# Tencent/FeatherCNN

Hardware: AMD Instinct MI355X
Metric: images/sec fp32 forward @224x224 (higher is better)
Workload: dtype f32; 1 GPU; vgg16 whole net (40 layers in the model file, 20 after fusion level 3), batch 32 per GPU, 224x224x3, fp32, synthetic ...; net=vgg16, mode=net, per_gpu_batch=32, global_batch=32, parallelism=batch-shard x1, launch=hipGraph replay per step, conv_routing=fhip_conv_select_algo_tuned

## Files before the change

feathercnn_amd/_lib.py:

```python
from __future__ import annotations

import collections
import ctypes
import functools
import os

_HERE = os.path.dirname(os.path.abspath(__file__))
_LOADED = {}

STAGE_NAMES = ("wino_input", "wino_gemm", "wino_output", "igemm", "depthwise", "init", "wino_chain")


class fhip_conv_param(ctypes.Structure):
    _fields_ = [(n, ctypes.c_int) for n in (
        "output_channels", "input_channels", "input_h", "input_w", "kernel_h", "kernel_w", "output_h", "output_w",
        "stride_h", "stride_w", "pad_left", "pad_bottom", "pad_right", "pad_top", "group", "bias_term", "activation")]


class fhip_winograd_plan(ctypes.Structure):
    _fields_ = [("tiles_x", ctypes.c_int), ("tiles_y", ctypes.c_int), ("tiles_per_image", ctypes.c_int),
                ("columns", ctypes.c_int), ("columns_padded", ctypes.c_int), ("column_block", ctypes.c_int), ("frequency_points", ctypes.c_int), ("tile_outputs", ctypes.c_int),
                ("in_channels_padded", ctypes.c_int),
                ("out_channels_padded", ctypes.c_int), ("v_offset_bytes", ctypes.c_size_t), ("v_bytes", ctypes.c_size_t),
                ("m_offset_bytes", ctypes.c_size_t), ("m_bytes", ctypes.c_size_t), ("u_bytes", ctypes.c_size_t)]
# ... 63 lines not shown
    "fhip_pooling_output_dim": (_I, [_Q, _PI, _PI]),
    "fhip_pooling": (_I, [_Q, _I, _V, _V, _V]),
    "fhip_softmax": (_I, [_V, _V, _I, _I, _V]),
    "fhip_net_create": (_I, [ctypes.POINTER(_V)]),
    "fhip_net_destroy": (_I, [_V]),
    "fhip_net_set_stream": (_I, [_V, _V]),
    "fhip_net_get_stream": (_I, [_V, ctypes.POINTER(_V)]),
    "fhip_net_set_fusion": (_I, [_V, _I]),
    "fhip_net_set_graph": (_I, [_V, _I]),
    "fhip_net_set_tuned_selection": (_I, [_V, _I]),
    "fhip_net_set_dilated": (_I, [_V, _I]),
    "fhip_net_set_quantized": (_I, [_V, _I]),
    "fhip_net_set_extended_layers": (_I, [_V, _I]),
    "fhip_net_set_concurrency": (_I, [_V, _I]),
    "fhip_net_set_sub_batches": (_I, [_V, _I]),
    "fhip_net_load_param": (_I, [_V, ctypes.c_char_p]),
    "fhip_net_load_param_mem": (_I, [_V, ctypes.c_char_p, _SZ]),
    "fhip_net_load_weights": (_I, [_V, ctypes.c_char_p]),
    "fhip_net_load_weights_mem": (_I, [_V, _V, _SZ]),
    "fhip_net_load_weights_device": (_I, [_V, _V, _SZ]),
    "fhip_net_feed_input": (_I, [_V, ctypes.c_char_p, _I, _I, _I, _I, _V, _I]),
    "fhip_net_feed_pixels": (_I, [_V, ctypes.c_char_p, _I, _V, _I, _I, _I, _I, _I, _V, _V, _I]),
    "fhip_net_feed_yuv420sp": (_I, [_V, ctypes.c_char_p, _I, _V, _I, _I, _I, _I, _I, _I, _V, _V, _I]),
    "fhip_net_feed_pixel_images": (_I, [_V, ctypes.c_char_p, _I, _V, _I, _I, _I, _V, _V, _I]),
    "fhip_net_forward": (_I, [_V]),
    "fhip_net_extract": (_I, [_V, ctypes.c_char_p, ctypes.POINTER(_V), _PI, _PI, _PI, _PI]),
    "fhip_net_extract_host": (_I, [_V, ctypes.c_char_p, _V, _SZ]),
    "fhip_net_layer_count": (_I, [_V]),
    "fhip_net_layer_info": (_I, [_V, _I, ctypes.c_char_p, ctypes.c_char_p, _I, _PI]),
    "fhip_net_layer_conv_param": (_I, [_V, _I, _P, _PI]),
    "fhip_net_layer_fused_pointwise": (_I, [_V, _I, _P, _PI]),
    "fhip_net_layer_chain": (_I, [_V, _I, _PI, _PI]),
    "fhip_net_layer_canvas": (_I, [_V, _I, _PI]),
    "fhip_net_layer_sibling": (_I, [_V, _I, _PI]),
    "fhip_net_layer_residual": (_I, [_V, _I, _PI]),
    "fhip_net_forward_timed": (_I, [_V, ctypes.POINTER(ctypes.c_float)]),
    "fhip_net_memory": (_I, [_V, ctypes.POINTER(_SZ), ctypes.POINTER(_SZ), ctypes.POINTER(_SZ)]),
}

PIXOUT_SIGNATURES = {
    "fhip_pixout_channels": (_I, [_I]),
    "fhip_float_to_pixels": (_I, [_V, _SZ, _V, _I, _I, _I, _I, _I, _I, _V, _V, _V]),
    "fhip_float_to_pixels_host": (_I, [_V, _SZ, _V, _I, _I, _I, _I, _I, _I, _V, _V, _V]),
    "fhip_pixout_last_error": (ctypes.c_char_p, []),
}

GCONV_SIGNATURES = {
    "fhip_gconv_supported": (_I, [_P]),
    "fhip_gconv_get_buffer_size": (_I, [_P, _I, ctypes.POINTER(_SZ), ctypes.POINTER(_SZ)]),
    "fhip_gconv_init": (_I, [_P, _V, _V, _V]),
    "fhip_gconv_forward": (_I, [_P, _I, _V, _V, _V, _V, _V, _V]),
    "fhip_gconv_route": (_I, [_P, _V, _V, ctypes.c_char_p, _I]),
    "fhip_gconv_last_error": (ctypes.c_char_p, []),
}

class fhip_deconv_param(ctypes.Structure):
    _fields_ = [(n, ctypes.c_int) for n in ("output_channels", "input_channels", "input_h", "input_w", "kernel_h", "kernel_w", "output_h", "output_w",
                                            "stride_h", "stride_w", "pad_left", "pad_bottom", "pad_right", "pad_top", "group", "bias_term",
                                            "activation", "output_pad_right", "output_pad_bottom")]


_DP = ctypes.POINTER(fhip_deconv_param)
DECONV_SIGNATURES = {
    "fhip_deconv_assign_output_dim": (_I, [_DP]),
    "fhip_deconv_supported": (_I, [_DP]),
    "fhip_deconv_get_buffer_size": (_I, [_DP, _I, ctypes.POINTER(_SZ), ctypes.POINTER(_SZ)]),
# ... 183 lines not shown
```

feathercnn_amd/csrc/common.h:

```cpp
#pragma once

#include <hip/hip_runtime.h>
#include <stdint.h>

#include "feather_hip/feather_hip.h"

namespace fhip
{

typedef float f32x16 __attribute__((ext_vector_type(16)));
typedef float f32x4 __attribute__((ext_vector_type(4)));

constexpr int kXcds = 8;

int fail(int code, const char* msg);
int fail_hip(hipError_t e, const char* what);

#define FHIP_CHECK_HIP(expr)                                       \
    do                                                             \
    {                                                              \
        hipError_t e__ = (expr);                                   \
        if (e__ != hipSuccess) return ::fhip::fail_hip(e__, #expr); \
    } while (0)

struct StageTimer
{
    StageTimer(int stage, hipStream_t s);
    ~StageTimer();
    int stage;
    hipStream_t stream;
    int slot;
};

int pixel_channels(int type, int* cin, int* cout);
int yuv420sp_check(int type, int w, int h, int target_w, int target_h, int resize_first, int* cout);

int device_compute_units();
size_t device_lds_bytes();

inline int ceil_div(int a, int b) { return (a + b - 1) / b; }
inline int round_up(int a, int b) { return ceil_div(a, b) * b; }
inline size_t round_up_sz(size_t a, size_t b) { return (a + b - 1) / b * b; }

__device__ __forceinline__ int xcd_remap(int bid, int nwg)
{
    const int q = nwg / kXcds, r = nwg % kXcds;
    const int xcd = bid % kXcds, local = bid / kXcds;
    const int start = (xcd < r) ? xcd * (q + 1) : r * (q + 1) + (xcd - r) * q;
    return start + local;
}

__device__ __forceinline__ float apply_act(float v, bool relu) { return relu ? fmaxf(v, 0.f) : v; }

__device__ __forceinline__ float4 ldg4_nt(const float* p)
{
    const f32x4 v = __builtin_nontemporal_load(reinterpret_cast<const f32x4*>(p));
    return make_float4(v.x, v.y, v.z, v.w);
}
__device__ __forceinline__ void stg4_nt(float* p, float4 v)
{
    f32x4 w;
    w.x = v.x;
    w.y = v.y;
    w.z = v.z;
    w.w = v.w;
    __builtin_nontemporal_store(w, reinterpret_cast<f32x4*>(p));
}
#ifndef FHIP_ACT_NT
#define FHIP_ACT_NT 0
#endif
template <int FAMILY>
// ... 55 lines not shown
```

feathercnn_amd/csrc/implicit_gemm.hip:

```cpp
#include <string.h>

#include <algorithm>
#include <mutex>

#include "gemm_core.h"
#include "conv_gemm_policy.h"
#include "dwpw_band.h"
#include "stream_gemm.h"
#include "ip_stream.h"

namespace fhip
{

size_t depthwise_packed_floats(const fhip_conv_param& p, size_t* w12_offset);

using ConvShapeBig = GemmShape<128, 64, 16, 2, 2>;
using ConvShapeSmallM = GemmShape<64, 128, 16, 1, 4>;

static bool conv_small_m(int K) { return K <= 64; }
using ConvShapeNarrow = GemmShape<64, 32, 16, 2, 1, 8>;
static bool conv_narrow_n(long long ntot) { return ntot <= 32; }

static bool stream_eligible(const fhip_conv_param& p)
{
// ... 465 lines not shown
        if (passes <= 3) FHIP_SMALLC_LAUNCH(2, 3);
        else if (passes <= 7) FHIP_SMALLC_LAUNCH(2, 7);
        else FHIP_SMALLC_LAUNCH(2, 11);
    }
#undef FHIP_SMALLC_LAUNCH
    FHIP_CHECK_HIP(hipGetLastError());
    return FHIP_OK;
}

template <class Shape, int MODE, bool TWIN = false>
static void launch(const ConvGemmParams& g0, hipStream_t s)
{
    ConvGemmParams g = g0;
    g.m_tiles = g.Kp / Shape::BM;
    g.n_tiles = ceil_div(g.Ntot, Shape::BN);
    g.batches = g.split_k;
    unsigned grid = (unsigned)(g.batches * g.m_tiles * g.n_tiles);
    if (g.tail_nt0 > 0)
    {
        g.tail_main = g.m_tiles * g.tail_nt0;
        g.part_col0 = g.tail_nt0 * Shape::BN;
        g.part_ntot = (g.n_tiles - g.tail_nt0) * Shape::BN;
        grid = (unsigned)(g.tail_main + g.m_tiles * (g.n_tiles - g.tail_nt0) * g.split_k);
    }
    else
    {
        g.tail_main = 0;
        g.part_col0 = 0;
        g.part_ntot = g.Ntot;
    }
    hipLaunchKernelGGL((gemm_mfma_kernel<Shape, ConvGemmPolicy<MODE, TWIN>>), dim3(grid), dim3(Shape::THREADS), 0, s, g);
}

int igemm_forward(const fhip_conv_param& p, int batch, float* out, const float* in, const float* packed, const float* bias,
                  float* buffer, bool force_no_act, hipStream_t s, const float* residual)
{
    if (p.group > 1) return fail(FHIP_E_UNSUPPORTED, "implicit GEMM handles group == 1 only");
    if (batch < 1) return fail(FHIP_E_BADARG, "batch < 1");
    if (p.bias_term && !bias) return fail(FHIP_E_BADARG, "bias_term set but bias_arr is NULL");
    ConvGemmParams g;
    g.batches = 1;
    g.Wt = packed;
    g.in = in;
    g.out = out;
    g.out2 = nullptr;
    g.twin_rows = g.relu2 = 0;
    g.bias = bias;
    g.has_residual = residual != nullptr;
    g.residual_delta = residual ? reinterpret_cast<const char*>(residual) - reinterpret_cast<const char*>(out) : 0;
    g.C = p.input_channels;
    g.K = p.output_channels;
    g.H = p.input_h;
    g.W = p.input_w;
    g.OH = p.output_h;
    g.OW = p.output_w;
    g.SH = p.stride_h > 0 ? p.stride_h : 1;
    g.SW = p.stride_w > 0 ? p.stride_w : 1;
    g.PL = p.pad_left;
    g.PT = p.pad_top;
    g.KH = p.kernel_h;
    g.KW = p.kernel_w;
    g.Kd = g.C * g.KH * g.KW;
    int kdp;
    igemm_packed_dims(p, &kdp, &g.Kp);
    g.Kdp = kdp;
    g.bm = conv_small_m(g.K) ? 64 : 128;
// ... 20 lines not shown
        q.bias = bias;
        q.C = g.C;
        q.K = g.K;
        q.HW = g.OHW;
        const bool ragged = (g.OHW % 4) != 0;
        q.gpi = (g.OHW + 3) / 4;
        q.total_px = ragged ? (long long)batch * q.gpi * 4 : ntot;
        q.mgroups = g.K / 32;
        q.px_tiles = (int)((q.total_px + 127) / 128);
        const unsigned blocks = (unsigned)q.px_tiles * (unsigned)((q.mgroups + 3) / 4);
        StageTimer tm(FHIP_STAGE_IGEMM, s);
#define FHIP_STREAM(D_, B_, R_)                                                                                     \
    do                                                                                                              \
    {                                                                                                               \
        if (ragged) hipLaunchKernelGGL((stream_gemm_kernel<D_, B_, R_, true>), dim3(blocks), dim3(256), 0, s, q);   \
        else hipLaunchKernelGGL((stream_gemm_kernel<D_, B_, R_, false>), dim3(blocks), dim3(256), 0, s, q);         \
    } while (0)
        const int pick = ((g.C % 32) == 0 ? 4 : 0) | (g.has_bias ? 2 : 0) | (g.relu ? 1 : 0);
        switch (pick)
        {
            case 7: FHIP_STREAM(16, true, true); break;
            case 6: FHIP_STREAM(16, true, false); break;
            case 5: FHIP_STREAM(16, false, true); break;
            case 4: FHIP_STREAM(16, false, false); break;
            case 3: FHIP_STREAM(8, true, true); break;
            case 2: FHIP_STREAM(8, true, false); break;
            case 1: FHIP_STREAM(8, false, true); break;
            default: FHIP_STREAM(8, false, false); break;
        }
#undef FHIP_STREAM
        FHIP_CHECK_HIP(hipGetLastError());
        return FHIP_OK;
    }
    if (!residual && ip_profitable(p, batch))
    {
        if (!buffer) return fail(FHIP_E_BADARG, "this geometry streams its weight matrix in pieces and needs the scratch buffer GetBufferSize asked for");
        IpStreamParams q;
        q.wp = packed + (size_t)kdp * g.Kp + (stream_eligible(p) ? (size_t)g.K * g.C : 0);
        q.xq = buffer;
        q.partial = buffer + ip_xq_floats(p);
        q.K = g.K;
        q.Kg = ip_kg(p);
        q.KQ = ip_kq(p);
        q.S = ip_pieces(p);
        q.batch = batch;
        StageTimer tm(FHIP_STAGE_IGEMM, s);
        hipLaunchKernelGGL(ip_pack_input_kernel, dim3(ceil_div(q.KQ, kIpPackOctets)), dim3(256), 0, s, buffer, in, batch, g.C, q.KQ);
        hipLaunchKernelGGL(ip_stream_kernel<4>, dim3((unsigned)q.S * (unsigned)ceil_div(q.Kg, 4)), dim3(256), 0, s, q);
        hipLaunchKernelGGL(ip_reduce_kernel, dim3(ceil_div(g.K * batch, 256)), dim3(256), 0, s, out, q.partial, bias, g.K, batch, q.S, g.has_bias, g.relu);
        FHIP_CHECK_HIP(hipGetLastError());
        return FHIP_OK;
    }
    g.split_k = igemm_split(p, batch);
    g.tail_main = g.tail_nt0 = 0;
    if (g.split_k <= 1)
    {
        int pieces;
        g.tail_nt0 = igemm_tail(p, batch, &pieces);
        if (g.tail_nt0) g.split_k = pieces;
    }
    if (g.split_k > 1 && !buffer) return fail(FHIP_E_BADARG, "this geometry runs split-K and needs the scratch buffer GetBufferSize asked for");
    g.partial = buffer;
    g.k_tiles = kdp / kConvKTile;
    g.m_tiles = 0;

    const bool one = g.KH == 1 && g.KW == 1 && p.pad_left == 0 && p.pad_right == 0 && p.pad_top == 0 && p.pad_bottom == 0;
    int mode = 0;
    if (one) mode = (g.SH == 1 && g.SW == 1 && (g.OHW % 4) == 0) ? 2 : 1;
    if (ragged_1x1(p, batch))
    {
        mode = 5;
        g.rag_gpi = (g.OHW + 3) / 4;
        const long long slots = igemm_columns(p, batch);
        if (slots > 0x7fffff00LL) return fail(FHIP_E_BADARG, "N*Ho*Wo exceeds 32-bit column indices: more than 0x7fffff00 GEMM columns");
        g.Ntot = (int)slots;
    }
    const bool small = conv_small_m(g.K);
    StageTimer tm(FHIP_STAGE_IGEMM, s);
    if (conv_narrow_n(ntot))
    {
        if (mode == 2) launch<ConvShapeNarrow, 2>(g, s);
        else if (mode == 1) launch<ConvShapeNarrow, 1>(g, s);
        else launch<ConvShapeNarrow, 0>(g, s);
    }
    else if (small)
// ... 219 lines not shown
```

feathercnn_amd/csrc/ip_stream.h:

```cpp
#pragma once

#include "common.h"

namespace fhip
{

struct IpStreamParams
{
    const float* wp;
    const float* xq;
    float* partial;
    int K, Kg, KQ, S, batch;
};

__global__ __launch_bounds__(256) void ip_pack_weights_kernel(float* __restrict__ wp, const float* __restrict__ w, int K, int C, int Kg, int KQ)
{
    const long long i = (long long)blockIdx.x * 256 + threadIdx.x;
    if (i >= (long long)Kg * KQ * 64) return;
    const int lane = (int)(i & 63);
    const long long gq = i >> 6;
    const int q = (int)(gq % KQ), g = (int)(gq / KQ);
    const int m = 32 * g + (lane & 31), k0 = 8 * q + (lane >> 5);
    float v[4];
#pragma unroll
// ... 79 lines not shown
            }
#pragma unroll
            for (int u = 0; u < UNR; ++u)
            {
                av[u] = an[u];
                bv[u] = bn[u];
            }
        }
        a += (size_t)UNR * 64;
        b += (size_t)UNR * 64;
#pragma unroll
        for (int u = 0; u < UNR; ++u)
        {
            FHIP_IP_MFMA4(av[u], bv[u]);
        }
    }
    for (int u = 0; u < tail; ++u)
    {
        const f32x4 a1 = FHIP_IP_LDW(a + (size_t)u * 64), b1 = b[(size_t)u * 64];
        FHIP_IP_MFMA4(a1, b1);
    }
    const int n = lane & 31, half = lane >> 5;
    if (n >= p.batch) return;
    float* out = p.partial + ((size_t)s * p.K + 32 * g + 4 * half) * p.batch + n;
#pragma unroll
    for (int r = 0; r < 16; ++r)
    {
        const int row = (r & 3) + 8 * (r >> 2);
        if (32 * g + 4 * half + row < p.K) out[(size_t)row * p.batch] = acc0[r] + acc1[r];
    }
}
#undef FHIP_IP_MFMA4

__global__ __launch_bounds__(256) void ip_reduce_kernel(float* __restrict__ out, const float* __restrict__ partial, const float* __restrict__ bias, int K,
                                                        int batch, int S, int has_bias, int relu)
{
    const int i = blockIdx.x * 256 + threadIdx.x, total = K * batch;
    if (i >= total) return;
    const int m = i / batch, n = i - m * batch;
    float acc = 0.f;
    int s = 0;
    for (; s + 4 <= S; s += 4)
    {
        const float v0 = partial[(size_t)s * total + i], v1 = partial[(size_t)(s + 1) * total + i], v2 = partial[(size_t)(s + 2) * total + i],
                    v3 = partial[(size_t)(s + 3) * total + i];
        acc = (((acc + v0) + v1) + v2) + v3;
    }
    for (; s < S; ++s) acc += partial[(size_t)s * total + i];
    if (has_bias) acc += bias[m];
    if (relu) acc = fmaxf(acc, 0.f);
    out[(size_t)n * K + m] = acc;
}

}
```

feathercnn_amd/csrc/net.hip:

```cpp
#include "net_side.h"
#include "net_model.h"
#include "net_core.h"
#include "net_conv.h"
#include "net_layers.h"
#include "net_plan.h"

namespace fhip::net
{

static Layer* create_extended_layer(const std::string& type)
{
    if (type == "Interp") return new InterpLayer;
    if (type == "HardSwish") return new HardSwishLayer;
    if (type == "LRN") return new LRNLayer;
    return nullptr;
}

static Layer* create_layer(const std::string& type)
{
    if (type == "Input") return new InputLayer;
    if (type == "Convolution" || type == "ConvolutionDepthWise") return new ConvLayer;
    if (type == "Deconvolution" || type == "DeconvolutionDepthWise") return new DeconvLayer;
    if (type == "ReLU") return new ReluLayer;
    if (type == "InstanceNorm") return new InstanceNormLayer;
// ... 675 lines not shown

int fhip_net_layer_sibling(fhip_net* n, int index, int* state)
{
    NET_GUARD(n);
    if (index < 0 || index >= (int)n->impl.layers.size() || !state) return fail(FHIP_E_BADARG, "layer index out of range");
    *state = n->impl.layers[index]->sibling_state();
    return FHIP_OK;
}

int fhip_net_layer_residual(fhip_net* n, int index, int* state)
{
    NET_GUARD(n);
    if (index < 0 || index >= (int)n->impl.layers.size() || !state) return fail(FHIP_E_BADARG, "layer index out of range");
    *state = n->impl.layers[index]->residual_state();
    return FHIP_OK;
}

int fhip_net_layer_chain(fhip_net* n, int index, int* v_from_previous, int* writes_next_v)
{
    NET_GUARD(n);
    if (index < 0 || index >= (int)n->impl.layers.size() || !v_from_previous || !writes_next_v) return fail(FHIP_E_BADARG, "layer index out of range");
    n->impl.layers[index]->chain_state(v_from_previous, writes_next_v);
    return FHIP_OK;
}

int fhip_net_layer_canvas(fhip_net* n, int index, int* canvas)
{
    NET_GUARD(n);
    if (index < 0 || index >= (int)n->impl.layers.size() || !canvas) return fail(FHIP_E_BADARG, "layer index out of range");
    *canvas = n->impl.layers[index]->canvas_state();
    return FHIP_OK;
}

int fhip_net_forward_timed(fhip_net* n, float* ms)
{
    NET_GUARD(n);
    if (!ms) return fail(FHIP_E_BADARG, "null argument");
    if (!n->more.empty())
        return fail(FHIP_E_UNSUPPORTED, "per-layer timing of a net with sub-batch replicas: kernels of concurrent replicas share the chip, "
                                        "so their durations are not layer times -- time a net created without fhip_net_set_sub_batches");
    Net& net = n->impl;
    int rc = prepare(net);
    if (rc) return rc;
    const size_t L = net.layers.size();
    std::vector<hipEvent_t> ev(L + 1);
    for (auto& e : ev) FHIP_CHECK_HIP(hipEventCreate(&e));
    FHIP_CHECK_HIP(hipEventRecord(ev[0], net.stream));
    for (size_t i = 0; i < L && rc == 0; ++i)
    {
        rc = net.layers[i]->Forward(net.stream);
        (void)hipEventRecord(ev[i + 1], net.stream);
    }
    (void)hipStreamSynchronize(net.stream);
    if (rc == 0)
        for (size_t i = 0; i < L; ++i) (void)hipEventElapsedTime(&ms[i], ev[i], ev[i + 1]);
    for (auto& e : ev) (void)hipEventDestroy(e);
    return rc;
}

int fhip_net_memory(fhip_net* n, size_t* blob_bytes, size_t* weight_bytes, size_t* arena_bytes)
{
    NET_GUARD(n);
    size_t bb = 0, wb = 0;
    for (auto& kv : n->impl.blobs) bb += kv.second->capacity * sizeof(float);
    for (auto& b : n->impl.shadowed) bb += b->capacity * sizeof(float);
    for (auto& l : n->impl.layers) wb += l->weight_bytes();
// ... 18 lines not shown
```

feathercnn_amd/csrc/net_core.h:

```cpp
#pragma once
#include "net_model.h"

namespace fhip::net
{

struct Blob
{
    std::string name;
    int n = 0, c = 0, h = 0, w = 0;
    float* data = nullptr;
    size_t capacity = 0;
    Blob* alias = nullptr;
    bool fused_away = false;
    bool chained = false;

    size_t count() const { return (size_t)n * c * h * w; }
    int reshape(int n_, int c_, int h_, int w_)
    {
        n = n_;
        c = c_;
        h = h_;
        w = w_;
        alias = nullptr;
        if (chained && !data) return 0;
// ... 40 lines not shown
        {
            release();
            FHIP_CHECK_HIP(hipMalloc((void**)&d, std::max<size_t>(count, 1) * 4));
            bytes = count * 4;
        }
        if (count) FHIP_CHECK_HIP(hipMemcpyAsync(d, h, count * 4, hipMemcpyHostToDevice, s));
        return 0;
    }
    int resize(size_t nbytes)
    {
        if (bytes != nbytes)
        {
            release();
            FHIP_CHECK_HIP(hipMalloc((void**)&d, std::max<size_t>(nbytes, 4)));
            bytes = nbytes;
        }
        return 0;
    }
    void release()
    {
        if (d) (void)hipFree(d);
        d = nullptr;
        bytes = 0;
    }
    ~DeviceVec() { release(); }
};

struct Net;
struct ConvLayer;
struct PoolingLayer;
struct AffineLayer;
struct EltwiseLayer;
struct InterpLayer;

struct Layer
{
    std::string type, name;
    std::vector<Blob*> bottoms, tops;
    Net* net = nullptr;

    virtual ~Layer() {}
    virtual bool needs_weights() const { return false; }
    virtual ConvLayer* as_conv() { return nullptr; }
    virtual PoolingLayer* as_pooling() { return nullptr; }
    virtual AffineLayer* as_affine() { return nullptr; }
    virtual EltwiseLayer* as_eltwise() { return nullptr; }
    virtual InterpLayer* as_interp() { return nullptr; }
    virtual const float* relu_slope() const { return nullptr; }
    template <class Api, class Call>
    int side(const Api* api, const Call& call, int code = 0, const char* prefix = "") const
    {
        if (!api) return FHIP_E_UNSUPPORTED;
        const int rc = call(api);
        return rc ? failf(code ? code : rc, "layer %s: %s%s", name.c_str(), prefix, api->last_error()) : 0;
    }
    virtual int LoadParam(const ParamDict&) { return 0; }
    virtual int LoadWeights(ModelBin&) { return 0; }
    virtual int Reshape()
    {
        if (tops.size() != 1 || bottoms.size() != 1) return failf(NET_E_BASE_RESHAPE, "layer %s: base Reshape needs 1 bottom and 1 top", name.c_str());
        return tops[0]->reshape(bottoms[0]->n, bottoms[0]->c, bottoms[0]->h, bottoms[0]->w);
    }
    int reshape_with(const void* side_library) { return side_library ? Layer::Reshape() : FHIP_E_UNSUPPORTED; }
    virtual int Init(hipStream_t) { return 0; }
    virtual int Forward(hipStream_t) = 0;
    virtual int Fuse(Layer*, int ) { return 0; }
    virtual size_t weight_bytes() const { return 0; }
    virtual size_t arena_bytes() const { return 0; }
    virtual int algo() const { return -1; }
    virtual const fhip_conv_param* conv_param() const { return nullptr; }
    virtual const fhip_conv_param* fused_pointwise(int*) const { return nullptr; }
    virtual void chain_state(int* v_from_previous, int* writes_next_v) const { *v_from_previous = *writes_next_v = 0; }
    virtual int canvas_state() const { return 0; }
    virtual int sibling_state() const { return 0; }
    virtual int residual_state() const { return 0; }
};

static bool is_plain_relu(const Layer* l)
{
    const float* slope = l->relu_slope();
    return slope && *slope == 0.f;
// ... 75 lines not shown
```

feathercnn_amd/csrc/net_layers.h:

```cpp
#pragma once
#include "net_conv.h"

namespace fhip::net
{

struct InputLayer : Layer
{
    int Reshape() override { return 0; }
    int Forward(hipStream_t) override { return 0; }
};

struct InnerProductLayer : Layer
{
    fhip_conv_param p;
    size_t input_size = 0, output_size = 0, weight_data_size = 0;
    std::vector<float> w_host, b_host;
    DeviceVec packed, bias;
    size_t buffer_bytes = 0, packed_bytes = 0;
    BuiltFor built;
    bool quant = false;
    QuantRoute qr;

    InnerProductLayer() { memset(&p, 0, sizeof(p)); }
    bool needs_weights() const override { return true; }
    int LoadParam(const ParamDict& pd) override
    {
        output_size = pd.get(0, 0);
        p.bias_term = pd.get(1, 0);
        weight_data_size = pd.get(2, 0);
        if (pd.get(0, 0) < 1) return failf(NET_E_SHAPE, "layer %s: num_output must be positive", name.c_str());
        if (pd.get(2, 0) < 0 || weight_data_size % output_size)
            return failf(NET_E_SHAPE, "layer %s: weight_data_size is no whole number of rows of num_output", name.c_str());
        input_size = weight_data_size / output_size;
        p.input_channels = (int)input_size;
        p.output_channels = (int)output_size;
        p.input_h = p.input_w = p.kernel_h = p.kernel_w = p.stride_h = p.stride_w = p.group = 1;
        fhip_conv_assign_output_dim(&p);
        quant = qr.read_scale_term(pd) != 0 && net && net->quantized;
        if (quant && (qr.scale_term < 0 || qr.scale_term > 100))
            return failf(NET_E_UNKNOWN_LAYER, "layer %s: int8_scale_term %d (requantised int8 output) is not supported", name.c_str(), qr.scale_term);
        return 0;
    }
    int LoadWeights(ModelBin& mb) override
    {
        if (quant) return qr.load(this, mb, weight_data_size, (int)output_size, p.bias_term != 0);
        int rc = mb.load(weight_data_size, 0, w_host);
        if (rc) return rc;
        if (p.bias_term) rc = mb.load(output_size, 1, b_host);
        return rc;
    }
    int Reshape() override
    {
        const Blob* b = bottoms[0];
        const size_t per_image = (size_t)b->c * b->h * b->w;
        if (input_size != per_image)
            return failf(NET_E_SHAPE, "In Layer %s: Bottom %s data size %zu is inconsistant with expected input size %zu.", name.c_str(), b->name.c_str(), per_image, input_size);
        if (quant)
        {
            copy_geometry(qr.q, p);
            return qr.reshape(this);
        }
        int rc = tops[0]->reshape(b->n, (int)output_size, 1, 1);
        if (rc) return rc;
        return fhip_conv_get_buffer_size(&p, FHIP_IM2COL, b->n, &buffer_bytes, &packed_bytes);
    }
    int Init(hipStream_t s) override
    {
        if (quant) return qr.init(this, AffineFold(), s);
        if (built.done()) return 0;
        const int rc = init_main(p, FHIP_IM2COL, w_host, b_host, packed, packed_bytes, bias, s);
        if (rc) return rc;
        std::vector<float>().swap(w_host);
        built = BuiltFor{FHIP_IM2COL, 0, packed_bytes};
        return 0;
    }
    int Forward(hipStream_t s) override
    {
        if (quant) return qr.forward(this, s);
        return fhip_conv_forward(&p, FHIP_IM2COL, bottoms[0]->n, tops[0]->data, bottoms[0]->data, packed.d, (float*)net->arena.d,
                                 p.bias_term ? bias.d : nullptr, s);
    }
    int Fuse(Layer* next, int) override
    {
        if (!is_plain_relu(next)) return 0;
        p.activation = FHIP_ACT_RELU;
        return 1;
    }
    size_t weight_bytes() const override { return packed.bytes + bias.bytes + qr.bytes(); }
    size_t arena_bytes() const override { return buffer_bytes; }
    int algo() const override { return quant ? FHIP_NET_ROUTE_QCONV : FHIP_IM2COL; }
};

struct ReluLayer : Layer
{
    float slope = 0.f;
    int LoadParam(const ParamDict& pd) override
    {
        slope = pd.get(0, 0.f);
        return 0;
    }
    int Reshape() override { return slope == 0.f ? Layer::Reshape() : reshape_with(inorm_api()); }
    int Forward(hipStream_t s) override
    {
        if (slope == 0.f) return fhip_relu(tops[0]->data, bottoms[0]->data, bottoms[0]->count(), s);
        const Blob* b = bottoms[0];
        return side(inorm_api(), [&](const InormApi* api) {
            return api->activation(FHIP_ACTIVATION_LEAKY_RELU, tops[0]->data, b->data, b->n, b->c, b->h * b->w, slope, 0.f, nullptr, s);
        });
    }
    const float* relu_slope() const override { return &slope; }
};
// ... 966 lines not shown
        for (Blob* t : tops) t->share(bottoms[0]);
        return 0;
    }
    int Forward(hipStream_t) override { return 0; }
};

struct DropoutLayer : Layer
{
    float scale = 1.f;
    DeviceVec d_scale;
    int LoadParam(const ParamDict& pd) override
    {
        scale = pd.get(0, 1.f);
        return 0;
    }
    int Reshape() override
    {
        if (scale == 1.f)
        {
            tops[0]->share(bottoms[0]);
            return 0;
        }
        return Layer::Reshape();
    }
    int Init(hipStream_t s) override
    {
        if (scale == 1.f || d_scale.d) return 0;
        std::vector<float> v(bottoms[0]->c, scale);
        int rc = d_scale.upload(v.data(), v.size(), s);
        if (rc) return rc;
        FHIP_CHECK_HIP(hipStreamSynchronize(s));
        return 0;
    }
    int Forward(hipStream_t s) override
    {
        if (scale == 1.f) return 0;
        const Blob* b = bottoms[0];
        return fhip_affine(tops[0]->data, b->data, d_scale.d, nullptr, b->n, b->c, b->h * b->w, 0, s);
    }
};

}
```

feathercnn_amd/csrc/net_plan.h:

```cpp
#pragma once
#include "net_layers.h"

namespace fhip::net
{

static bool is_channel_map_type(const Layer* l)
{
    return l->type == "ShuffleChannel" || l->type == "Slice" || (l->type == "Concat" && static_cast<const ConcatLayer*>(l)->axis == 0);
}

static void collapse_channel_maps(Net& net)
{
    auto holds = [](const std::vector<Blob*>& v, const Blob* b) { return std::find(v.begin(), v.end(), b) != v.end(); };
    for (size_t i = 0; i < net.layers.size(); ++i)
    {
        if (!is_channel_map_type(net.layers[i].get())) continue;
        std::vector<Blob*> made = net.layers[i]->tops;
        size_t end = i + 1;
        for (; end < net.layers.size(); ++end)
        {
            const Layer* l = net.layers[end].get();
            if (!is_channel_map_type(l)) break;
            bool reads = false, sole = true;
            for (const Blob* b : l->bottoms)
// ... 365 lines not shown
    }
    net.chain_slot[0] = 0;
    net.chain_slot[1] = slot[0];
    net.chain_m = slot[0] + slot[1];
    for (ConvLayer* c : conv)
        if (c && c->chain.runs()) c->chain.arena(slot[0] + slot[1] + msz);
    return 0;
}

static int plan_siblings(Net& net)
{
    const size_t L = net.layers.size();
    std::vector<ConvLayer*> conv(L, nullptr);
    for (size_t i = 0; i < L; ++i)
        if (net.layers[i]->type != "ConvolutionDepthWise" && (conv[i] = net.layers[i]->as_conv())) conv[i]->sibs.reset();
    if (net.fusion < 2) return 0;
    auto root = [](const Blob* b) { return b->alias ? b->alias : b; };
    auto plain = [](const ConvLayer* c) { return c && c->unclaimed() && c->algo_ == FHIP_IM2COL && c->tops.size() == 1 && c->bottoms.size() == 1; };
    auto pairs = [&](const ConvLayer* a, const ConvLayer* b) {
        if (!plain(a) || !plain(b) || root(a->bottoms[0]) != root(b->bottoms[0]) || a->tops[0] == b->tops[0]) return false;
        if (a->p.output_channels <= 64 || b->p.output_channels <= 64) return false;
        return fhip_conv_can_fuse_siblings(&a->p, a->algo_, &b->p, b->algo_, a->bottoms[0]->n) != 0;
    };
    for (size_t i = 0; i < L; ++i)
    {
        if (i + 1 < L && pairs(conv[i], conv[i + 1]))
            SiblingPlan::pair(conv[i], conv[i + 1]);
        else if (conv[i])
            conv[i]->sibs.unpaired();
    }
    return 0;
}

static int reshape_all(Net& net)
{
    net.drop_graph();
    size_t need = 0;
    for (auto& l : net.layers)
    {
        const int rc = l->Reshape();
        if (rc) return rc;
    }
    {
        int rc = plan_chains(net);
        if (rc) return rc;
        if ((rc = plan_siblings(net))) return rc;
    }
    for (auto& l : net.layers) need = std::max(need, l->arena_bytes());
    if (need > net.arena.bytes)
    {
        const int rc = net.arena.resize(need);
        if (rc) return rc;
    }
    net.shapes_dirty = false;
    return plan_concurrency(net);
}

static int prepare(Net& net)
{
    if (!net.param_loaded) return failf(NET_E_IO, "Network has not been loaded. Please load the param file first.");
    if (!net.weights_loaded)
    {
        bool needs = false;
        for (auto& l : net.layers) needs = needs || l->needs_weights();
        if (needs) return failf(NET_E_IO, "weights have not been loaded");
    }
    fuse_layers(net);
    for (auto& kv : net.blobs)
        if (!kv.second->fused_away && kv.second->count() == 0)
        {
            bool is_input = false;
            for (auto& l : net.layers)
                if (l->type == "Input")
                    for (Blob* tb : l->tops) is_input = is_input || tb == kv.second.get();
            if (is_input) return failf(NET_E_SHAPE, "input blob %s has not been fed", kv.first.c_str());
        }
    if (net.shapes_dirty)
    {
        const int rc = reshape_all(net);
        if (rc) return rc;
    }
    for (auto& l : net.layers)
    {
        const int rc = l->Init(net.stream);
        if (rc) return rc;
    }
    net.initialized = true;
    return 0;
// ... 52 lines not shown
```

feathercnn_amd/net.py:

```python
from __future__ import annotations

import ctypes

import numpy as np

from . import _lib
from .booster import ALGO_NAMES, FeatherHipError, _check, _stream


ROUTE_GCONV = 100
ROUTE_NAMES = dict(ALGO_NAMES)
ROUTE_NAMES[ROUTE_GCONV] = "GCONV"
ROUTE_DECONV = 101
ROUTE_NAMES[ROUTE_DECONV] = "DECONV"
ROUTE_INORM = 102
ROUTE_NAMES[ROUTE_INORM] = "INORM"
ROUTE_SHUFFLE = 103
ROUTE_NAMES[ROUTE_SHUFFLE] = "SHUFFLE"
ROUTE_ATROUS = 104
ROUTE_NAMES[ROUTE_ATROUS] = "ATROUS"
ROUTE_GATE = 105
ROUTE_NAMES[ROUTE_GATE] = "GATE"
ROUTE_RESAMPLE = 106
ROUTE_NAMES[ROUTE_RESAMPLE] = "RESAMPLE"
# ... 201 lines not shown
        for i in range(self._lib.fhip_net_layer_count(self._h)):
            st = ctypes.c_int()
            if self._lib.fhip_net_layer_sibling(self._h, i, ctypes.byref(st)) == 0 and st.value:
                out[i] = st.value
        return out

    def residuals(self):
        out = {}
        for i in range(self._lib.fhip_net_layer_count(self._h)):
            st = ctypes.c_int()
            if self._lib.fhip_net_layer_residual(self._h, i, ctypes.byref(st)) == 0 and st.value:
                out[i] = st.value
        return out

    def chains(self, raw=False):
        out = {}
        for i in range(self._lib.fhip_net_layer_count(self._h)):
            a, b = ctypes.c_int(), ctypes.c_int()
            if self._lib.fhip_net_layer_chain(self._h, i, ctypes.byref(a), ctypes.byref(b)) == 0 and (a.value or b.value):
                if raw:
                    out[i] = (a.value, b.value)
                elif a.value == 1 or b.value == 1:
                    out[i] = (a.value == 1, b.value == 1)
        return out

    def canvases(self):
        out = []
        for i in range(self._lib.fhip_net_layer_count(self._h)):
            c = ctypes.c_int()
            if self._lib.fhip_net_layer_canvas(self._h, i, ctypes.byref(c)) == 0 and c.value:
                out.append(i)
        return out

    def forward_timed(self):
        n = self._lib.fhip_net_layer_count(self._h)
        ms = (ctypes.c_float * max(n, 1))()
        _check(self._lib.fhip_net_forward_timed(self._h, ms), "fhip_net_forward_timed")
        info = self.layers()
        return [(t, nm, a, ms[i]) for i, (t, nm, a) in enumerate(info)]

    def memory(self):
        v = [ctypes.c_size_t() for _ in range(3)]
        _check(self._lib.fhip_net_memory(self._h, *[ctypes.byref(x) for x in v]), "fhip_net_memory")
        return {"blob_bytes": v[0].value, "weight_bytes": v[1].value, "arena_bytes": v[2].value}


def _p(t):
    return ctypes.c_void_p(t.data_ptr()) if t is not None else None


def relu(x):
    import torch
    y = torch.empty_like(x)
    _check(_lib.load_library().fhip_relu(_p(y), _p(x), x.numel(), _stream()), "fhip_relu")
    return y


def add(a, b, relu: bool = False):
    import torch
    y = torch.empty_like(a)
    _check(_lib.load_library().fhip_add(_p(y), _p(a), _p(b), a.numel(), int(relu), _stream()), "fhip_add")
    return y


def affine(x, mul, add_=None, relu: bool = False):
    import torch
# ... 29 lines not shown
```

include/feather_hip/feather_net.h:

```cpp
#ifndef FEATHER_NET_H_
#define FEATHER_NET_H_

#include "feather_hip/feather_hip.h"

#ifdef __cplusplus
extern "C" {
#endif


FHIP_API int fhip_relu(float* y, const float* x, size_t count, void* stream);

FHIP_API int fhip_add(float* y, const float* a, const float* b, size_t count, int relu, void* stream);

FHIP_API int fhip_affine(float* y, const float* x, const float* mul, const float* add, int batch, int channels, int hw,
                         int relu, void* stream);


enum
{
    FHIP_PIXEL_CONVERT_SHIFT = 16,
    FHIP_PIXEL_RGB = 1,
    FHIP_PIXEL_BGR = (1 << 1),
    FHIP_PIXEL_GRAY = (1 << 2),
    FHIP_PIXEL_RGBA = (1 << 3),
// ... 88 lines not shown
FHIP_API int fhip_net_load_param(fhip_net* net, const char* path);
FHIP_API int fhip_net_load_param_mem(fhip_net* net, const char* text, size_t len);
FHIP_API int fhip_net_load_weights(fhip_net* net, const char* path);
FHIP_API int fhip_net_load_weights_mem(fhip_net* net, const void* data, size_t len);
FHIP_API int fhip_net_load_weights_device(fhip_net* net, const void* device_data, size_t len);

FHIP_API int fhip_net_feed_input(fhip_net* net, const char* blob_name, int n, int c, int h, int w, const float* data,
                                 int on_device);
FHIP_API int fhip_net_feed_pixels(fhip_net* net, const char* blob_name, int n, const unsigned char* pixels, int type, int w, int h,
                                  int target_w, int target_h, const float* mean, const float* norm, int on_device);
FHIP_API int fhip_net_feed_yuv420sp(fhip_net* net, const char* blob_name, int n, const unsigned char* yuv, int w, int h, int target_w,
                                    int target_h, int type, int resize_first, const float* mean, const float* norm, int on_device);
FHIP_API int fhip_net_feed_pixel_images(fhip_net* net, const char* blob_name, int n, const fhip_pixel_image* images, int type,
                                        int target_w, int target_h, const float* mean, const float* norm, int on_device);
FHIP_API int fhip_net_forward(fhip_net* net);
FHIP_API int fhip_net_extract(fhip_net* net, const char* blob_name, float** device_ptr, int* n, int* c, int* h, int* w);
FHIP_API int fhip_net_extract_host(fhip_net* net, const char* blob_name, float* host, size_t capacity);

FHIP_API int fhip_net_layer_count(fhip_net* net);
#define FHIP_NET_ROUTE_GCONV 100
#define FHIP_NET_ROUTE_DECONV 101
#define FHIP_NET_ROUTE_INORM 102
#define FHIP_NET_ROUTE_SHUFFLE 103
#define FHIP_NET_ROUTE_ATROUS 104
#define FHIP_NET_ROUTE_GATE 105
#define FHIP_NET_ROUTE_RESAMPLE 106
#define FHIP_NET_ROUTE_LRN 107
#define FHIP_NET_ROUTE_QCONV 108
FHIP_API int fhip_net_layer_info(fhip_net* net, int index, char* type, char* name, int len, int* algo);
FHIP_API int fhip_net_layer_conv_param(fhip_net* net, int index, fhip_conv_param* param, int* batch);
FHIP_API int fhip_net_layer_fused_pointwise(fhip_net* net, int index, fhip_conv_param* param, int* one_kernel);
FHIP_API int fhip_net_layer_chain(fhip_net* net, int index, int* v_from_previous, int* writes_next_v);
FHIP_API int fhip_net_layer_canvas(fhip_net* net, int index, int* canvas);
FHIP_API int fhip_net_layer_sibling(fhip_net* net, int index, int* state);
FHIP_API int fhip_net_layer_residual(fhip_net* net, int index, int* state);
FHIP_API int fhip_net_forward_timed(fhip_net* net, float* ms);
FHIP_API int fhip_net_memory(fhip_net* net, size_t* blob_bytes, size_t* weight_bytes, size_t* arena_bytes);

#ifdef __cplusplus
}
#endif
#endif
```

Baseline: 10270 images/s.

## Hand over packed inner-product input directly from reduce kernel to next FC layer

When two streaming inner-product layers follow each other (optionally through pass-through layers like dropout), the first layer's reduce kernel now also writes its output in the packed layout the next layer expects. The next layer then skips its input-packing kernel. This removes one kernel launch and a read/write pass per FC pair in VGG16's classifier head. In exchange the reduce kernel does extra scattered stores, and it relies on planning checks so the arena scratch is not clobbered between the two layers.

```diff
diff --git a/feathercnn_amd/_lib.py b/feathercnn_amd/_lib.py
--- a/feathercnn_amd/_lib.py
+++ b/feathercnn_amd/_lib.py
@@ -119,6 +119,7 @@
     "fhip_net_layer_fused_pointwise": (_I, [_V, _I, _P, _PI]),
     "fhip_net_layer_chain": (_I, [_V, _I, _PI, _PI]),
     "fhip_net_layer_canvas": (_I, [_V, _I, _PI]),
+    "fhip_net_layer_handover": (_I, [_V, _I, _PI, _PI]),
     "fhip_net_layer_sibling": (_I, [_V, _I, _PI]),
     "fhip_net_layer_residual": (_I, [_V, _I, _PI]),
     "fhip_net_forward_timed": (_I, [_V, ctypes.POINTER(ctypes.c_float)]),
diff --git a/feathercnn_amd/csrc/common.h b/feathercnn_amd/csrc/common.h
--- a/feathercnn_amd/csrc/common.h
+++ b/feathercnn_amd/csrc/common.h
@@ -37,6 +37,17 @@
 
 int device_compute_units();
 size_t device_lds_bytes();
+
+struct IpHandover
+{
+    bool packed_in = false;
+    float* next_xq = nullptr;
+    int next_kq = 0;
+};
+bool ip_streams(const fhip_conv_param& p, int batch);
+size_t ip_xq_bytes(const fhip_conv_param& p);
+int ip_forward(const fhip_conv_param& p, int batch, float* out, const float* in, const float* packed, const float* bias, float* buffer, hipStream_t s,
+               const IpHandover& h);
 
 inline int ceil_div(int a, int b) { return (a + b - 1) / b; }
 inline int round_up(int a, int b) { return ceil_div(a, b) * b; }
diff --git a/feathercnn_amd/csrc/implicit_gemm.hip b/feathercnn_amd/csrc/implicit_gemm.hip
--- a/feathercnn_amd/csrc/implicit_gemm.hip
+++ b/feathercnn_amd/csrc/implicit_gemm.hip
@@ -521,6 +521,43 @@
     hipLaunchKernelGGL((gemm_mfma_kernel<Shape, ConvGemmPolicy<MODE, TWIN>>), dim3(grid), dim3(Shape::THREADS), 0, s, g);
 }
 
+static int ip_launch(const fhip_conv_param& p, int batch, float* out, const float* in, const float* packed, const float* bias, float* buffer, bool relu,
+                     hipStream_t s, const IpHandover& h)
+{
+    if (!buffer) return fail(FHIP_E_BADARG, "this geometry streams its weight matrix in pieces and needs the scratch buffer GetBufferSize asked for");
+    int kdp, kp;
+    igemm_packed_dims(p, &kdp, &kp);
+    const int K = p.output_channels, C = p.input_channels;
+    IpStreamParams q;
+    q.wp = packed + (size_t)kdp * kp + (stream_eligible(p) ? (size_t)K * C : 0);
+    q.xq = buffer;
+    q.partial = buffer + ip_xq_floats(p);
+    q.K = K;
+    q.Kg = ip_kg(p);
+    q.KQ = ip_kq(p);
+    q.S = ip_pieces(p);
+    q.batch = batch;
+    if (h.next_xq && h.next_kq != ceil_div(K, 8)) return fail(FHIP_E_BADARG, "the next layer's packed input does not have this layer's output width");
+    StageTimer tm(FHIP_STAGE_IGEMM, s);
+    if (!h.packed_in) hipLaunchKernelGGL(ip_pack_input_kernel, dim3(ceil_div(q.KQ, kIpPackOctets)), dim3(256), 0, s, buffer, in, batch, C, q.KQ);
+    hipLaunchKernelGGL(ip_stream_kernel<4>, dim3((unsigned)q.S * (unsigned)ceil_div(q.Kg, 4)), dim3(256), 0, s, q);
+    const int reduce_threads = h.next_xq ? h.next_kq * 256 : K * batch;
+    hipLaunchKernelGGL(ip_reduce_kernel, dim3(ceil_div(reduce_threads, 256)), dim3(256), 0, s, out, q.partial, bias, K, batch, q.S, p.bias_term != 0, relu ? 1 : 0,
+                       h.next_xq, h.next_kq);
+    FHIP_CHECK_HIP(hipGetLastError());
+    return FHIP_OK;
+}
+
+bool ip_streams(const fhip_conv_param& p, int batch) { return ip_profitable(p, batch); }
+size_t ip_xq_bytes(const fhip_conv_param& p) { return ip_xq_floats(p) * sizeof(float); }
+int ip_forward(const fhip_conv_param& p, int batch, float* out, const float* in, const float* packed, const float* bias, float* buffer, hipStream_t s,
+               const IpHandover& h)
+{
+    if (!ip_profitable(p, batch) || !out || !packed || (!in && !h.packed_in)) return fail(FHIP_E_BADARG, "bad argument");
+    if (p.bias_term && !bias) return fail(FHIP_E_BADARG, "bias_term set but bias_arr is NULL");
+    return ip_launch(p, batch, out, in, packed, bias, buffer, p.activation == FHIP_ACT_RELU, s, h);
+}
+
 int igemm_forward(const fhip_conv_param& p, int batch, float* out, const float* in, const float* packed, const float* bias,
                   float* buffer, bool force_no_act, hipStream_t s, const float* residual)
 {
@@ -607,25 +644,7 @@
         FHIP_CHECK_HIP(hipGetLastError());
         return FHIP_OK;
     }
-    if (!residual && ip_profitable(p, batch))
-    {
-        if (!buffer) return fail(FHIP_E_BADARG, "this geometry streams its weight matrix in pieces and needs the scratch buffer GetBufferSize asked for");
-        IpStreamParams q;
-        q.wp = packed + (size_t)kdp * g.Kp + (stream_eligible(p) ? (size_t)g.K * g.C : 0);
-        q.xq = buffer;
-        q.partial = buffer + ip_xq_floats(p);
-        q.K = g.K;
-        q.Kg = ip_kg(p);
-        q.KQ = ip_kq(p);
-        q.S = ip_pieces(p);
-        q.batch = batch;
-        StageTimer tm(FHIP_STAGE_IGEMM, s);
-        hipLaunchKernelGGL(ip_pack_input_kernel, dim3(ceil_div(q.KQ, kIpPackOctets)), dim3(256), 0, s, buffer, in, batch, g.C, q.KQ);
-        hipLaunchKernelGGL(ip_stream_kernel<4>, dim3((unsigned)q.S * (unsigned)ceil_div(q.Kg, 4)), dim3(256), 0, s, q);
-        hipLaunchKernelGGL(ip_reduce_kernel, dim3(ceil_div(g.K * batch, 256)), dim3(256), 0, s, out, q.partial, bias, g.K, batch, q.S, g.has_bias, g.relu);
-        FHIP_CHECK_HIP(hipGetLastError());
-        return FHIP_OK;
-    }
+    if (!residual && ip_profitable(p, batch)) return ip_launch(p, batch, out, in, packed, bias, buffer, g.relu, s, IpHandover());
     g.split_k = igemm_split(p, batch);
     g.tail_main = g.tail_nt0 = 0;
     if (g.split_k <= 1)
diff --git a/feathercnn_amd/csrc/ip_stream.h b/feathercnn_amd/csrc/ip_stream.h
--- a/feathercnn_amd/csrc/ip_stream.h
+++ b/feathercnn_amd/csrc/ip_stream.h
@@ -135,12 +135,9 @@
 }
 #undef FHIP_IP_MFMA4
 
-__global__ __launch_bounds__(256) void ip_reduce_kernel(float* __restrict__ out, const float* __restrict__ partial, const float* __restrict__ bias, int K,
-                                                        int batch, int S, int has_bias, int relu)
+__device__ __forceinline__ float ip_reduce_value(const float* __restrict__ partial, const float* __restrict__ bias, int i, int m, int total, int S, int has_bias,
+                                                 int relu)
 {
-    const int i = blockIdx.x * 256 + threadIdx.x, total = K * batch;
-    if (i >= total) return;
-    const int m = i / batch, n = i - m * batch;
     float acc = 0.f;
     int s = 0;
     for (; s + 4 <= S; s += 4)
@@ -152,7 +149,29 @@
     for (; s < S; ++s) acc += partial[(size_t)s * total + i];
     if (has_bias) acc += bias[m];
     if (relu) acc = fmaxf(acc, 0.f);
-    out[(size_t)n * K + m] = acc;
+    return acc;
+}
+
+__global__ __launch_bounds__(256) void ip_reduce_kernel(float* __restrict__ out, const float* __restrict__ partial, const float* __restrict__ bias, int K,
+                                                        int batch, int S, int has_bias, int relu, float* __restrict__ xq_next, int KQ_next)
+{
+    const int i = blockIdx.x * 256 + threadIdx.x, total = K * batch;
+    if (xq_next)
+    {
+        if (i >= KQ_next * 256) return;
+        const int n = i & 31, m = i >> 5;
+        float v = 0.f;
+        if (n < batch && m < K)
+        {
+            v = ip_reduce_value(partial, bias, m * batch + n, m, total, S, has_bias, relu);
+            out[(size_t)n * K + m] = v;
+        }
+        xq_next[((size_t)(m >> 3) * 64 + n + 32 * (m & 1)) * 4 + ((m & 7) >> 1)] = v;
+        return;
+    }
+    if (i >= total) return;
+    const int m = i / batch, n = i - m * batch;
+    out[(size_t)n * K + m] = ip_reduce_value(partial, bias, i, m, total, S, has_bias, relu);
 }
 
 }
diff --git a/feathercnn_amd/csrc/net.hip b/feathercnn_amd/csrc/net.hip
--- a/feathercnn_amd/csrc/net.hip
+++ b/feathercnn_amd/csrc/net.hip
@@ -731,6 +731,16 @@
     return FHIP_OK;
 }
 
+int fhip_net_layer_handover(fhip_net* n, int index, int* packed_in, int* writes_next)
+{
+    NET_GUARD(n);
+    if (index < 0 || index >= (int)n->impl.layers.size() || !packed_in || !writes_next) return fail(FHIP_E_BADARG, "layer index out of range");
+    const InnerProductLayer* ip = n->impl.layers[index]->as_inner_product();
+    *packed_in = ip && ip->hand.packed_in ? 1 : 0;
+    *writes_next = ip && ip->hand.next_kq ? 1 : 0;
+    return FHIP_OK;
+}
+
 int fhip_net_forward_timed(fhip_net* n, float* ms)
 {
     NET_GUARD(n);
diff --git a/feathercnn_amd/csrc/net_core.h b/feathercnn_amd/csrc/net_core.h
--- a/feathercnn_amd/csrc/net_core.h
+++ b/feathercnn_amd/csrc/net_core.h
@@ -96,6 +96,7 @@
 struct AffineLayer;
 struct EltwiseLayer;
 struct InterpLayer;
+struct InnerProductLayer;
 
 struct Layer
 {
@@ -110,7 +111,9 @@
     virtual AffineLayer* as_affine() { return nullptr; }
     virtual EltwiseLayer* as_eltwise() { return nullptr; }
     virtual InterpLayer* as_interp() { return nullptr; }
+    virtual InnerProductLayer* as_inner_product() { return nullptr; }
     virtual const float* relu_slope() const { return nullptr; }
+    virtual bool passes_through() const { return false; }
     template <class Api, class Call>
     int side(const Api* api, const Call& call, int code = 0, const char* prefix = "") const
     {
diff --git a/feathercnn_amd/csrc/net_layers.h b/feathercnn_amd/csrc/net_layers.h
--- a/feathercnn_amd/csrc/net_layers.h
+++ b/feathercnn_amd/csrc/net_layers.h
@@ -20,9 +20,12 @@
     BuiltFor built;
     bool quant = false;
     QuantRoute qr;
+    IpHandover hand;
 
     InnerProductLayer() { memset(&p, 0, sizeof(p)); }
     bool needs_weights() const override { return true; }
+    InnerProductLayer* as_inner_product() override { return this; }
+    bool streams() const { return !quant && ip_streams(p, bottoms[0]->n); }
     int LoadParam(const ParamDict& pd) override
     {
         output_size = pd.get(0, 0);
@@ -77,6 +80,12 @@
     int Forward(hipStream_t s) override
     {
         if (quant) return qr.forward(this, s);
+        if (hand.packed_in || hand.next_kq)
+        {
+            IpHandover h = hand;
+            if (h.next_kq) h.next_xq = (float*)net->arena.d;
+            return ip_forward(p, bottoms[0]->n, tops[0]->data, bottoms[0]->data, packed.d, p.bias_term ? bias.d : nullptr, (float*)net->arena.d, s, h);
+        }
         return fhip_conv_forward(&p, FHIP_IM2COL, bottoms[0]->n, tops[0]->data, bottoms[0]->data, packed.d, (float*)net->arena.d,
                                  p.bias_term ? bias.d : nullptr, s);
     }
@@ -1109,6 +1118,7 @@
         FHIP_CHECK_HIP(hipStreamSynchronize(s));
         return 0;
     }
+    bool passes_through() const override { return scale == 1.f; }
     int Forward(hipStream_t s) override
     {
         if (scale == 1.f) return 0;
diff --git a/feathercnn_amd/csrc/net_plan.h b/feathercnn_amd/csrc/net_plan.h
--- a/feathercnn_amd/csrc/net_plan.h
+++ b/feathercnn_amd/csrc/net_plan.h
@@ -421,6 +421,36 @@
     return 0;
 }
 
+static void plan_handovers(Net& net)
+{
+    const size_t L = net.layers.size();
+    for (auto& l : net.layers)
+        if (InnerProductLayer* ip = l->as_inner_product()) ip->hand = IpHandover();
+    if (net.fusion < 3) return;
+    auto main_stream = [&](size_t i) { return i >= net.side.size() || net.side[i] < 0; };
+    for (size_t i = 0; i < L; ++i)
+    {
+        InnerProductLayer* a = net.layers[i]->as_inner_product();
+        if (!a || a->tops.size() != 1 || a->bottoms.size() != 1 || !a->streams() || !main_stream(i)) continue;
+        const Blob* t = a->tops[0];
+        int j = readers(net, t, i + 1).sole();
+        while (j >= 0 && net.layers[j]->passes_through() && net.layers[j]->tops.size() == 1)
+        {
+            t = net.layers[j]->tops[0];
+            j = readers(net, t, j + 1).sole();
+        }
+        InnerProductLayer* b = j >= 0 ? net.layers[j]->as_inner_product() : nullptr;
+        if (!b || b->bottoms.size() != 1 || b->bottoms[0] != t || !b->streams() || !main_stream(j)) continue;
+        if (b->bottoms[0]->n != a->bottoms[0]->n || b->input_size != a->output_size) continue;
+        if (ip_xq_bytes(b->p) > ip_xq_bytes(a->p)) continue;
+        bool arena_free = true;
+        for (int k = (int)i + 1; k < j; ++k) arena_free = arena_free && net.layers[k]->arena_bytes() == 0;
+        if (!arena_free) continue;
+        a->hand.next_kq = (int)((a->output_size + 7) / 8);
+        b->hand.packed_in = true;
+    }
+}
+
 static int reshape_all(Net& net)
 {
     net.drop_graph();
@@ -442,7 +472,9 @@
         if (rc) return rc;
     }
     net.shapes_dirty = false;
-    return plan_concurrency(net);
+    const int rc = plan_concurrency(net);
+    if (!rc) plan_handovers(net);
+    return rc;
 }
 
 static int prepare(Net& net)
diff --git a/feathercnn_amd/net.py b/feathercnn_amd/net.py
--- a/feathercnn_amd/net.py
+++ b/feathercnn_amd/net.py
@@ -257,6 +257,14 @@
                 out.append(i)
         return out
 
+    def handovers(self):
+        out = {}
+        for i in range(self._lib.fhip_net_layer_count(self._h)):
+            a, b = ctypes.c_int(), ctypes.c_int()
+            if self._lib.fhip_net_layer_handover(self._h, i, ctypes.byref(a), ctypes.byref(b)) == 0 and (a.value or b.value):
+                out[i] = (bool(a.value), bool(b.value))
+        return out
+
     def forward_timed(self):
         n = self._lib.fhip_net_layer_count(self._h)
         ms = (ctypes.c_float * max(n, 1))()
diff --git a/include/feather_hip/feather_net.h b/include/feather_hip/feather_net.h
--- a/include/feather_hip/feather_net.h
+++ b/include/feather_hip/feather_net.h
@@ -144,6 +144,7 @@
 FHIP_API int fhip_net_layer_fused_pointwise(fhip_net* net, int index, fhip_conv_param* param, int* one_kernel);
 FHIP_API int fhip_net_layer_chain(fhip_net* net, int index, int* v_from_previous, int* writes_next_v);
 FHIP_API int fhip_net_layer_canvas(fhip_net* net, int index, int* canvas);
+FHIP_API int fhip_net_layer_handover(fhip_net* net, int index, int* packed_in, int* writes_next);
 FHIP_API int fhip_net_layer_sibling(fhip_net* net, int index, int* state);
 FHIP_API int fhip_net_layer_residual(fhip_net* net, int index, int* state);
 FHIP_API int fhip_net_forward_timed(fhip_net* net, float* ms);
```

Result: no change. 10290 images/s, median of 4 (+0.1%).
